# sclipman/gfa2network

Hardware: AMD Instinct MI355X
Metric: M edges/sec GFA->CSR (device-resident), + GB/s ingested (higher is better)
Workload: dtype u8/int64 (float64 weights); 1 GPU; C4: 50M S / 200M L, default (directed, MAX-SYM CSR), HBM-resident parse; n_segments=50000000, n_links=200000000, input_bytes_per_gpu=6299989066, n_nodes=50000000, nnz=289480899, mode=default, output=csr, parallelism=replica x1

## Files before the change

### gfa2network_amd/_native.py

```python
from __future__ import annotations

import ctypes
import os
import sys
from dataclasses import dataclass, field
from pathlib import Path

import numpy as np

LIB_PATH = Path(__file__).resolve().parent / "_lib" / "libg2n.so"

ABI_VERSION = 2
MAX_PHASES = 40

OK = 0
E_MALFORMED_L, E_MALFORMED_E, E_MALFORMED_C, E_MALFORMED_P, E_MALFORMED_O = 1, 2, 3, 4, 5
E_INDEX_LIST, E_INDEX_BYTES, E_UNICODE, E_INT_TOO_LARGE = 6, 7, 8, 9
E_CAST_OVERFLOW, E_CAST_INF, E_CAST_NAN = 10, 11, 12
E_ARG, E_IO, E_GZIP, E_DEVICE, E_NOMEM, E_UNSUPPORTED = 13, 14, 15, 16, 17, 18

DTYPE_CODES = {"bool": 0, "int8": 1, "int32": 2, "float32": 3, "float64": 4}
CODE_DTYPES = {v: np.dtype(k) for k, v in DTYPE_CODES.items()}
OUT_PARSE, OUT_CSR, OUT_COO, OUT_EDGE_LIST = 0, 1, 2, 3
FMT_COO, FMT_CSR, FMT_TEXT = 0, 1, 2

EXPORTED = [
    "g2n_version", "g2n_abi_version", "g2n_options_init", "g2n_device_count", "g2n_device_memory", "g2n_last_error",
    "g2n_status_name", "g2n_release_shared", "g2n_build_from_path", "g2n_build_from_buffer", "g2n_result_free",
    "g2n_coo_to_csr", "g2n_coo_to_csr_band", "g2n_context_create", "g2n_context_destroy", "g2n_context_stream", "g2n_context_trim",
    "g2n_build_device", "g2n_build_decimal_range", "g2n_count_device", "g2n_order_keys", "g2n_rank_keys", "g2n_upload_file_range", "g2n_partition_keys", "g2n_dedup_keys", "g2n_gather_keys", "g2n_remap_pairs", "g2n_route_triplets", "g2n_csr_from_coo_pair",
    "g2n_context_group_slots", "g2n_route_group_slots", "g2n_csr_from_group_slots",
    "g2n_keyset_create", "g2n_keyset_add", "g2n_keyset_view", "g2n_keyset_free",
    "g2n_gunzip", "g2n_gunzip_chunked", "g2n_free", "g2n_split_render", "g2n_split_get", "g2n_split_segments", "g2n_split_free", "g2n_join_names", "g2n_gather_names", "g2n_write_npz", "g2n_write_node_map", "g2n_first_bad_utf8",
    "g2n_csr_stats", "g2n_csr_stats_host", "g2n_stats_from_path",
    "g2n_csr_path_distances", "g2n_csr_path_distances_host", "g2n_load_paths", "g2n_paths_get", "g2n_paths_free",
    "g2n_distances_from_path", "g2n_csr_path_distances_weighted", "g2n_csr_path_distances_weighted_host",
    "g2n_seq_distance_from_path", "g2n_seq_hits_get", "g2n_seq_hits_names", "g2n_seq_hits_free",
]


TEST_NO_BUCKETS = 2
TEST_NO_LEAN = 4
TEST_DICT_HASH = 8
TEST_DICT_GENERAL = 16
TEST_NO_TILE_LOCAL = 32
TEST_HOST_INFLATE = 64
TEST_NO_GROUP = 128
TEST_NO_HASH_LEAN = 256
TEST_THROW_AFTER_IDS = 512
TEST_INDEX64 = 1024
TEST_DICT_DIRECT = 2048
TEST_NO_DIRECT = 4096
TEST_NO_EXT_LEAN = 8192
TEST_NO_DEC_TEXT = 16384
TEST_NO_DEC_PREFIX = 32768
TEST_FLAGS = int(os.environ.get("G2N_TEST_FLAGS", "0"), 0)
RANGE_DECIMAL = 1
RANGE_EVIDENCE = 2
RANGE_NO_VALUES = 4
RANGE_SLOTS = 8


class Options(ctypes.Structure):
    _fields_ = [
        ("abi_version", ctypes.c_uint32),
        ("directed", ctypes.c_int32),
        ("bidirected", ctypes.c_int32),
        ("keep_directed_bidir", ctypes.c_int32),
        ("asymmetric", ctypes.c_int32),
        ("strip_orientation", ctypes.c_int32),
        ("dtype", ctypes.c_int32),
        ("output", ctypes.c_int32),
        ("weight_tag", ctypes.c_char_p),
        ("want_node_names", ctypes.c_int32),
        ("device", ctypes.c_int32),
        ("unknown_warned", ctypes.c_int32),
        ("range_flags", ctypes.c_int32),
        ("range_s_base", ctypes.c_int64),
        ("range_n_segments", ctypes.c_int64),
        ("test_flags", ctypes.c_uint32),
        ("reserved_", ctypes.c_int32 * 3),
    ]


class Result(ctypes.Structure):
    _fields_ = [
        ("abi_version", ctypes.c_uint32),
        ("status", ctypes.c_int32),
        ("err_line", ctypes.c_int64),
        ("err_index", ctypes.c_int64),
        ("err_value", ctypes.c_double),
        ("err_detail", ctypes.c_void_p),
        ("err_detail_len", ctypes.c_int64),
        ("has_warning", ctypes.c_int32),
        ("warn_byte", ctypes.c_int32),
        ("warn_line", ctypes.c_int64),
        ("n_lines", ctypes.c_int64),
        ("n_records", ctypes.c_int64),
        ("n_records_before_error", ctypes.c_int64),
        ("n_edges", ctypes.c_int64),
        ("n_nodes", ctypes.c_int64),
        ("names_blob", ctypes.c_void_p),
        ("names_offsets", ctypes.c_void_p),
        ("format", ctypes.c_int32),
        ("dtype", ctypes.c_int32),
        ("index_width", ctypes.c_int32),
        ("sum_sorted", ctypes.c_int32),
        ("nnz", ctypes.c_int64),
# ... 291 lines not shown
    o.device = int(device)
    o.test_flags = int(TEST_FLAGS if test_flags is None else test_flags)
    return o


class _Owner:

    def __init__(self, ptr):
        self.ptr = ptr

    def __del__(self):
        if self.ptr is not None and _lib is not None:
            _lib.g2n_result_free(self.ptr)
            self.ptr = None


def _view(addr: int | None, count: int, dtype, owner: _Owner) -> np.ndarray:
    dtype = np.dtype(dtype)
    if not addr or count == 0:
        return np.zeros(0, dtype=dtype)
    buf = (ctypes.c_uint8 * (count * dtype.itemsize)).from_address(addr)
    buf._g2n_owner = owner
    return np.frombuffer(buf, dtype=dtype, count=count)


@dataclass
class RawResult:

    status: int = 0
    message: str = ""
    err_line: int = -1
    err_index: int = -1
    err_value: float = 0.0
    err_detail: bytes = b""
    has_warning: bool = False
    warn_byte: int = 0
    warn_line: int = -1
    n_lines: int = 0
    n_records: int = 0
    n_records_before_error: int = 0
    n_edges: int = 0
    n_nodes: int = 0
    names_blob: np.ndarray | None = None
    names_offsets: np.ndarray | None = None
    format: str = "coo"
    dtype: np.dtype = field(default_factory=lambda: np.dtype("float64"))
    rows: np.ndarray | None = None
    cols: np.ndarray | None = None
    indptr: np.ndarray | None = None
    indices: np.ndarray | None = None
    data: np.ndarray | None = None
    sum_sorted: bool = True
    sum_buckets: bool = False
    n_cast_overflow: int = 0
    input_bytes: int = 0
    phase_ms: dict = field(default_factory=dict)
    host_ms: dict = field(default_factory=dict)


def _from_result(ptr, rc: int) -> RawResult:
    if not ptr:
        raise RuntimeError(f"{status_name(rc)}: {last_error()}")
    r = ptr.contents
    owner = _Owner(ptr)
    out = RawResult(status=r.status, message=last_error() if r.status else "")
    out.err_line, out.err_index, out.err_value = r.err_line, r.err_index, r.err_value
    if r.err_detail and r.err_detail_len:
        out.err_detail = ctypes.string_at(r.err_detail, r.err_detail_len)
    out.has_warning, out.warn_byte, out.warn_line = bool(r.has_warning), r.warn_byte, r.warn_line
    out.n_lines, out.n_records = r.n_lines, r.n_records
    out.n_records_before_error, out.n_edges, out.n_nodes = r.n_records_before_error, r.n_edges, r.n_nodes
    out.dtype = CODE_DTYPES.get(r.dtype, np.dtype("float64"))
    out.sum_sorted = bool(r.sum_sorted)
    out.sum_buckets = r.sum_sorted < 0
    out.n_cast_overflow = int(r.n_cast_overflow)
    out.input_bytes = int(r.input_bytes)
    if r.format == FMT_TEXT and r.data:
        out.format = "text"
        out.data = _view(r.data, r.nnz, np.uint8, owner)
    elif r.status == OK:
        idx = np.int32 if r.index_width == 4 else np.int64
        if r.names_offsets:
            out.names_offsets = _view(r.names_offsets, r.n_nodes + 1, np.int64, owner)
            out.names_blob = _view(r.names_blob, int(out.names_offsets[-1]), np.uint8, owner)
        if r.format == FMT_COO:
            out.format = "coo"
            out.rows = _view(r.rows, r.nnz, idx, owner)
            out.cols = _view(r.cols, r.nnz, idx, owner)
        else:
            out.format = "csr"
            out.indptr = _view(r.indptr, r.n_nodes + 1, idx, owner)
            out.indices = _view(r.indices, r.nnz, idx, owner)
        out.data = _view(r.data, r.nnz, out.dtype, owner)
    for k in range(r.n_phases):
        name = r.phase_names[k].decode()
        if not name.startswith("_"):
            out.phase_ms[name] = out.phase_ms.get(name, 0.0) + r.phase_ms[k]
    out.host_ms = {"read": r.host_ms_read, "h2d": r.host_ms_h2d, "d2h": r.host_ms_d2h}
    return out


def build_from_path(path: str, opts: Options) -> RawResult:
    lib = load()
    res = ctypes.POINTER(Result)()
    rc = lib.g2n_build_from_path(os.fsencode(path), ctypes.byref(opts), ctypes.byref(res))
    return _from_result(res, rc)


def build_from_buffer(data: bytes | bytearray | memoryview | np.ndarray, opts: Options) -> RawResult:
    lib = load()
    arr = np.frombuffer(data, dtype=np.uint8) if not isinstance(data, np.ndarray) else data
    arr = np.ascontiguousarray(arr, dtype=np.uint8)
    res = ctypes.POINTER(Result)()
    rc = lib.g2n_build_from_buffer(arr.ctypes.data if arr.size else None, arr.size, ctypes.byref(opts),
                                   ctypes.byref(res))
    return _from_result(res, rc)


def _stats_dict(st: GraphStats) -> dict:
    return {"n_nodes": int(st.n_nodes), "n_entries": int(st.n_entries), "n_diag": int(st.n_diag),
            "n_components": int(st.n_components), "max_degree": int(st.max_degree),
            "ms_degree": float(st.ms_degree), "ms_components": float(st.ms_components)}


def stats_from_path(path: str, opts: Options) -> tuple[RawResult, dict, int]:
    lib = load()
    res = ctypes.POINTER(Result)()
# ... 494 lines not shown
```

### gfa2network_amd/csrc/g2n_kernels.h

```cpp
#pragma once
#include <hip/hip_runtime.h>
#include <stdint.h>

#include "stl_sort.h"

namespace g2n {

constexpr int kTPB = 256;
constexpr uint64_t kTile = 32768;
constexpr uint32_t kTileHalo = 2048;

enum : uint8_t { kSkip = 0, kUnknown = 1, kS = 2, kEdge = 3, kPO = 4 };

enum : uint32_t {
  kErrMalformedL = 1,
  kErrMalformedE = 2,
  kErrMalformedC = 3,
  kErrMalformedP = 4,
  kErrMalformedO = 5,
  kErrIndexList = 6,
  kErrIndexBytes = 7,
  kErrUnicode = 8,
  kErrIntTooLarge = 9,
  kErrCastOverflow = 10,
  kErrCastInf = 11,
  kErrCastNan = 12,
};

constexpr uint64_t kConstFlag = 1ull << 62;
constexpr unsigned long long kEmptySlot = ~0ull;

struct Ctl {
  unsigned long long err_key;
  unsigned long long warn_line;
  unsigned long long cast_key;
  unsigned long long wl_count;
  unsigned long long n_lines;
  unsigned long long n_records;
  unsigned long long n_edges;
  unsigned long long n_s;
  unsigned long long n_records_before;
  unsigned long long n_nodes;
  unsigned long long names_len;
  unsigned long long table_overflow;
  unsigned long long detail_off;
  unsigned long long detail_len;
  unsigned long long unsorted[2];
  unsigned long long flagged[2];
  unsigned long long n_unique[2];
  unsigned long long n_keep;
  unsigned long long n_f32_overflow;
  unsigned long long deferred;
  unsigned long long dict_general;
  unsigned long long s_late;
  unsigned long long row_gap;
  unsigned long long n_deferred;
  unsigned long long int_fail;
  unsigned long long bucket_overflow;
  unsigned long long bad_id;
  unsigned long long ev_dmin, ev_dmax;
  unsigned long long ev_vmax;
  unsigned long long w_inexact;
  unsigned long long warn_tile;
  unsigned long long warn_off;
  unsigned long long dir_vmax;
};

struct ParseOpts {
  int bidir, keep, strip, has_wt;
  uint32_t wt_len;
  const uint8_t* wt;
  uint32_t* tid;
  uint64_t n_seg;
  uint64_t s_base;
  int32_t* rows;
  int32_t* cols;
  uint32_t ktrip;
  uint32_t tile_pad;
  uint32_t grouped;
  double* ew;
  uint64_t wt_pack;
  uint32_t* tunk;
  uint64_t dpre;
  uint32_t dpre_len;
  uint32_t gshift;
  uint32_t* wenc;
  uint32_t wf32;
};
constexpr uint32_t kGroupShift = 5;

struct TileLean {
  long long dmin, dmax;
  unsigned long long vmax;
};

struct TouchOut {
  uint64_t* noff;
  uint32_t* nlen;
  uint64_t* ooff;
  uint32_t* olen;
  uint8_t* tkind;
};
struct DictEntry {
  unsigned long long hdr;
  unsigned long long meta;
  unsigned long long k0, k1;
};
struct TouchIn {
  const uint64_t* noff;
  const uint32_t* nlen;
  const uint64_t* ooff;
// ... 35 lines not shown
```

### gfa2network_amd/csrc/g2n_pipeline.hip

```cpp
#include <hip/hip_runtime.h>

#include <chrono>
#include <cstring>
#include <functional>
#include <map>
#include <memory>
#include <mutex>

#include "g2n_internal.h"
#include "g2n_kernels.hip"
#include "g2n_scan.hip"
#include "g2n_sort.hip"
#include "g2n_sym.hip"
#include "g2n_route.hip"
#include "g2n_inflate.hip"
#include "g2n_keyset.hip"
#include "g2n_stats.hip"
#include "g2n_dist.hip"
#include "g2n_wdist.hip"
#include "g2n_seq.hip"

#define G2N_HIP(call)                                                                                      \
  do {                                                                                                     \
    hipError_t e_ = (call);                                                                                \
    if (e_ != hipSuccess)                                                                                  \
      throw ::g2n::Failure(G2N_E_DEVICE, std::string(#call " failed: ") + hipGetErrorString(e_));          \
  } while (0)

namespace g2n {

enum Slot {
  S_IN, S_TILE_CNT, S_TILE_BASE, S_LS, S_KIND, S_NOFF, S_NLEN, S_OOFF, S_OLEN, S_EW, S_ETB, S_WL, S_TABLE,
  S_SLOT, S_FIRST, S_NID, S_FLEN, S_BLOB, S_OFFS, S_ROWS, S_COLS, S_DATA, S_KEYS0, S_KEYS1, S_VALS0, S_VALS1,
  S_KV, S_ODATA, S_INDPTR, S_INDICES, S_TEMP, S_WT, S_TKIND, S_TSTATE, S_RSTART0, S_RSTART1, S_ROUT0,
  S_ROUT1, S_UCNT0, S_UCNT1, S_UOFF, S_MCNT, S_MOFF, S_RSCR, S_RFLAG0, S_RFLAG1, S_RVAL0, S_RVAL1, S_TID,
  S_INV, S_TUNK, S_DEFER, S_FOFF64, S_BTC, S_BTV, S_BTOT, S_EBAD, S_ELEN, S_EPOS, S_ETEXT, S_EFIRST, S_EMETA, S_EL0, S_EL1,
  S_PCNT, S_POFF, S_PGRP, S_BSTART, S_SCANST, S_RBOUND, S_ROWSP, S_COLSP, S_TLEAN, S_ZIN, S_ZMEM, S_ZBAD, S_RSK, S_RSV, S_RSCNT, S_RSOFF,
  S_GCNT, S_TCN, S_INDPTR64, S_INDICES64, S_WENC, S_W1, S_W2, S_TVAL, S_PW0, S_PW1, S_BSTARTA, S_DIRECT, S_RTOT, S_SCANST2, S_EWP, S_TLIST, S_TNB, S_WENCP,
  S_STPARENT, S_STCOL, S_STDIAG, S_STLONG, S_STOUT, S_STIP, S_STIX,
  S_DSEEN, S_DNEXT, S_DQUEUE, S_DQMASK, S_DLONG, S_DSTATE, S_DCNT, S_DMPTR, S_DCUR, S_DMPATH, S_DSPATH, S_DDONE,
  S_DTAB, S_DPP, S_DPN,
  S_WDIST, S_WVAL,
  S_DFLAG, S_DKS, S_DSBLOB, S_DSOFFS, S_DIDS,
  S_QSTATE, S_QLINES, S_QNODE, S_QFPOS, S_QFLAG, S_QLAST, S_QCAND, S_QIDS, S_QBYTES, S_QNLEN, S_QNOFF, S_QNBLOB,
  S_NSLOTS
};

constexpr uint64_t kMinGroups = 1024;
constexpr uint32_t kPtileSmallDiv = 4;
constexpr uint32_t kF2Ranges = 4;
constexpr uint32_t kTestNoBuckets = G2N_TEST_NO_BUCKETS;
constexpr uint32_t kTestNoLean = G2N_TEST_NO_LEAN;
constexpr uint32_t kTestDictHash = G2N_TEST_DICT_HASH;
constexpr uint32_t kTestDictGeneral = G2N_TEST_DICT_GENERAL;
constexpr uint32_t kTestNoTileLocal = G2N_TEST_NO_TILE_LOCAL;
constexpr uint32_t kTestNoGroup = G2N_TEST_NO_GROUP;
constexpr uint32_t kTestNoHashLean = G2N_TEST_NO_HASH_LEAN;
constexpr uint32_t kTestThrowAfterIds = G2N_TEST_THROW_AFTER_IDS;
constexpr uint32_t kTestIndex64 = G2N_TEST_INDEX64;
constexpr uint32_t kTestDictDirect = G2N_TEST_DICT_DIRECT;
constexpr uint32_t kTestNoDirect = G2N_TEST_NO_DIRECT;
constexpr uint32_t kTestNoExtLean = G2N_TEST_NO_EXT_LEAN;
constexpr uint32_t kTestNoDecText = G2N_TEST_NO_DEC_TEXT;
constexpr uint32_t kTestNoDecPrefix = G2N_TEST_NO_DEC_PREFIX;


struct DevBuf {
  void* p = nullptr;
  size_t cap = 0;
  uint64_t call = 0;
};
struct ScanSlot {
  void* p = nullptr;
  size_t cap = 0;
  uint32_t epoch = 0;
  uint64_t ticket = 0;
};

struct GroupedCoo {
  bool active = false;
  bool failed = false;
  const int32_t* rows = nullptr;
  const int32_t* cols = nullptr;
  const uint32_t* gcount = nullptr;
  uint64_t gcap = 0, n_groups = 0;
  const uint32_t* wenc = nullptr;
};

}

struct g2n_context {
  int device = 0;
  int n_cu = 256;
  uint32_t test_flags = 0;
  uint64_t err_line_off = 0;
  g2n::GroupedCoo gcoo;
  g2n::GroupedCoo slots;
  const uint32_t* wenc = nullptr;
  bool no_group = false;
  g2n::ScanSlot scan_slot[g2n::S_NSLOTS];
  bool edge_text = false;
  bool names_dec = false;
  bool stats_names = false;
  uint64_t last_n_segs = 0;
  hipStream_t stream = nullptr;
  hipStream_t side = nullptr;
  hipEvent_t side_ev[2] = {nullptr, nullptr};
  hipStream_t place = nullptr;
  hipEvent_t ov_ev[17] = {};
  bool side_pending = false;
  bool range_has_s = false;
  int64_t range_d = -1;
  uint64_t range_vmax = 0;
  uint64_t range_nseg = 0;
  std::function<void()> side_work;
  std::vector<g2n::DevBuf> bufs;
  uint64_t call_id = 0;
// ... 362 lines not shown
    const uint64_t n_blk2 = (n_el + ptile - 1) / ptile + n_dig1;
    const uint64_t n2 = (uint64_t)n_dig2 * n_blk2;
    const uint64_t ns = words ? 2 : 1;
    auto* cnt2 = dget<uint32_t>(c, S_PCNT, ns * n2);
    auto* off2 = dget<uint32_t>(c, S_POFF, std::max<uint64_t>(ns * n2, ns * nm1));
    auto* el2 = dget<uint2>(c, S_EL1, n_el);
    PartSrc s2a{nullptr, nullptr, 0, 0, nullptr, nullptr, 0, 0, nullptr, grpA, grpA + n_dig1 + 1, n_dig1,
                nullptr, 0, (uint32_t)low + 1u, nullptr, wa1, ptile};
    s2a.obase = off2 + n2;
    uint16_t* wa2 = words ? dget<uint16_t>(c, S_PW1, n_trip) : nullptr;
    const bool wide = bits2 > (int)kMaxDigitBits;
    if (wide) {
      hipLaunchKernelGGL((k_part_hist<2, kWideDigitBits>), dim3((unsigned)n_blk2), dim3(kPartTPB), 0, c->stream, s2,
                         (uint32_t)low, n_dig2, cnt2, n_blk2);
      if (words)
        hipLaunchKernelGGL((k_part_hist<7, kWideDigitBits>), dim3((unsigned)n_blk2), dim3(kPartTPB), 0, c->stream,
                           s2a, 2u * (uint32_t)low, n_dig2, cnt2 + n2, n_blk2);
    } else {
      hipLaunchKernelGGL(k_part_hist<2>, dim3((unsigned)n_blk2), dim3(kPartTPB), 0, c->stream, s2, (uint32_t)low,
                         n_dig2, cnt2, n_blk2);
      if (words)
        hipLaunchKernelGGL(k_part_hist<7>, dim3((unsigned)n_blk2), dim3(kPartTPB), 0, c->stream, s2a,
                           2u * (uint32_t)low, n_dig2, cnt2 + n2, n_blk2);
    }
    scan_excl<uint32_t, uint32_t>(c, cnt2, off2, ns * n2);
    if (wide)
      hipLaunchKernelGGL((k_part_scatter<2, kWideDigitBits>), dim3((unsigned)n_blk2), dim3(kPartTPB), 0, c->stream, s2,
                         (uint32_t)low, n_dig2, (const uint32_t*)off2, n_blk2, el2);
    else
      hipLaunchKernelGGL(k_part_scatter<2>, dim3((unsigned)n_blk2), dim3(kPartTPB), 0, c->stream, s2, (uint32_t)low,
                         n_dig2, (const uint32_t*)off2, n_blk2, el2);
    hipLaunchKernelGGL(k_part_bucket_starts, dim3(grid_for(n_buckets + 1)), dim3(kTPB), 0, c->stream,
                       (const uint32_t*)off2, s2, n_dig2, n_buckets, bst);
    el = el2;
    if (words) {
      if (wide)
        hipLaunchKernelGGL((k_part_scatter<7, kWideDigitBits>), dim3((unsigned)n_blk2), dim3(kPartTPB), 0,
                           c->stream, s2a, 2u * (uint32_t)low, n_dig2, (const uint32_t*)(off2 + n2), n_blk2,
                           (uint2*)nullptr, (uint32_t*)wa2);
      else
        hipLaunchKernelGGL(k_part_scatter<7>, dim3((unsigned)n_blk2), dim3(kPartTPB), 0, c->stream, s2a,
                           2u * (uint32_t)low, n_dig2, (const uint32_t*)(off2 + n2), n_blk2, (uint2*)nullptr,
                           (uint32_t*)wa2);
      hipLaunchKernelGGL(k_part_bucket_starts, dim3(grid_for(n_buckets + 1)), dim3(kTPB), 0, c->stream,
                         (const uint32_t*)(off2 + n2), s2a, n_dig2, n_buckets, bstA);
      wa = wa2;
    }
  }
  phase(c, "sum");
  auto* indptr = dget<int32_t>(c, S_INDPTR, n_rows + 1);
  auto* indices = dget<int32_t>(c, S_INDICES, n_el);
  T* odata = dget<T>(c, S_ODATA, n_el);
  auto* btot = dget<uint32_t>(c, S_BTOT, n_bk);
  uint2* tmp = el == el1 ? dget<uint2>(c, S_EL1, n_el) : el1;
  auto* tcol = (uint32_t*)tmp;
  auto* tcn = dget<uint16_t>(c, S_TCN, 2 * n_el);
  G2N_HIP(hipMemsetAsync(&c->ctl->bucket_overflow, 0, sizeof(unsigned long long), c->stream));
#ifdef G2N_F1_STAMPS
  unsigned long long* f1st = dget<unsigned long long>(c, S_TEMP, n_bk * kF1Stamps);
  G2N_HIP(hipMemsetAsync(f1st, 0, n_bk * kF1Stamps * 8, c->stream));
  G2N_HIP(hipMemcpyToSymbolAsync(HIP_SYMBOL(g2n_f1_stamps), &f1st, sizeof(f1st), 0, hipMemcpyHostToDevice,
                                 c->stream));
#endif
  fork_side(c);
  const uint32_t n_ov = (n_el <= 0x7FFFFFFFull && !(c->test_flags & kTestIndex64) && n_bk >= 32768ull) ? kF2Ranges : 1u;
  auto rb = [&](uint32_t k) -> uint64_t { return n_bk * k / n_ov; };
  uint32_t* boff = nullptr;
  auto launch_f1 = [&](uint64_t b0, uint64_t nb) {
    auto* f1 = sum ? k_sym_finish<T, true> : k_sym_finish<T, false>;
    hipLaunchKernelGGL(f1, dim3((unsigned)nb), dim3(kFinTPB), 0, c->stream, el, (const uint32_t*)bst, (uint32_t)low,
                       n_rows, (T)1, btot, tcol, tcn, indptr, c->ctl, (uint32_t)row_base, wa, (const uint32_t*)bstA,
                       (uint32_t)b0);
  };
  auto launch_f2 = [&](hipStream_t st, auto* ind, int64_t* ip64, uint64_t b0, uint64_t nb, const uint32_t* rt,
                       uint32_t rk) {
    using I = std::remove_pointer_t<decltype(ind)>;
    hipLaunchKernelGGL((k_sym_place<T, I>), dim3((unsigned)nb), dim3(kFinTPB), 0, st, (const uint32_t*)bst,
                       (const uint32_t*)btot, (const uint32_t*)boff, (uint32_t)low, n_rows, (T)1, (const uint32_t*)tcol,
                       (const uint16_t*)tcn, indptr, ind, odata, ip64, (const uint32_t*)bstA, (uint32_t)b0, rt, rk);
  };
  if (n_ov > 1) {
    boff = dget<uint32_t>(c, S_MOFF, n_bk + 1);
    auto* rtot = dget<uint32_t>(c, S_RTOT, n_ov);
    (void)dget<unsigned long long>(c, S_SCANST2, scan_tiles(n_bk) + 1);
    for (uint32_t k = 0; k < n_ov; k++) {
      launch_f1(rb(k), rb(k + 1) - rb(k));
      G2N_HIP(hipEventRecord(c->ov_ev[k], c->stream));
    }
    for (uint32_t k = 0; k < n_ov; k++) {
      const uint64_t b0 = rb(k), b1 = rb(k + 1);
      G2N_HIP(hipStreamWaitEvent(c->place, c->ov_ev[k], 0));
      scan_excl<uint32_t, uint32_t>(c, (const uint32_t*)(btot + b0), boff + b0, b1 - b0, rtot + k, c->place, S_SCANST2);
      launch_f2(c->place, indices, nullptr, b0, b1 - b0, rtot, k);
    }
    G2N_HIP(hipEventRecord(c->ov_ev[16], c->place));
    G2N_HIP(hipStreamWaitEvent(c->stream, c->ov_ev[16], 0));
    int32_t nnz = 0;
    G2N_HIP(hipMemcpyAsync(&nnz, indptr + n_rows, sizeof(int32_t), hipMemcpyDeviceToHost, c->stream));
    sync_ctl(c);
#ifdef G2N_F1_STAMPS
    stamps_to_file(c, "G2N_F1_STAMPS_OUT", f1st, n_bk / n_ov * kF1Stamps);
#endif
    if (c->h_ctl->bucket_overflow) return false;
    R->format = G2N_FMT_CSR;
    R->indptr = indptr;
    R->nnz = (int64_t)nnz;
    R->indices = indices;
    R->data = odata;
    R->sum_sorted = -1;
    R->sum_t_sorted = -1;
    phase(c, sum ? "csr" : "maxsym");
    return true;
  }
  launch_f1(0, n_bk);
#ifdef G2N_F1_STAMPS
  stamps_to_file(c, "G2N_F1_STAMPS_OUT", f1st, n_bk * kF1Stamps);
#endif
  boff = dget<uint32_t>(c, S_MOFF, n_bk + 1);
  scan_excl<uint32_t, uint32_t>(c, btot, boff, n_bk, boff + n_bk);
  if (n_el > 0x7FFFFFFFull || (c->test_flags & kTestIndex64)) {
    sync_ctl(c);
    if (c->h_ctl->bucket_overflow) return false;
  }
  const bool wide = (c->test_flags & kTestIndex64) || (sum && !pair && n_trip > 0x7FFFFFFFull) ||
                    (!sum && n_el > 0x7FFFFFFFull && (uint64_t)read_dev(c, boff + n_bk) > 0x7FFFFFFFull);
  if (wide) {
// ... 2417 lines not shown
```

### gfa2network_amd/csrc/g2n_sym.hip

```cpp
#pragma once
#include <hip/hip_runtime.h>
#include <stdint.h>

#include <type_traits>

#include "g2n_kernels.h"
#include "g2n_scan.hip"
#include "g2n_symword.h"

namespace g2n {

constexpr uint32_t kPartTPB = 1024;
constexpr uint32_t kSubPer = 8;
constexpr uint32_t kSub = kSubPer * kPartTPB;
constexpr uint32_t kChunkSubs = 8 * 1024 / kPartTPB;
constexpr uint32_t kPartTile = kSub * kChunkSubs;
constexpr uint32_t kMaxDigitBits = 10;
constexpr uint32_t kWideDigitBits = 11;
constexpr uint32_t kFinTPB = 256;
static_assert(kFinTPB == 1u << kSymLowMax, "a finish bucket's row must fit the 8-bit fields of a 16-bit pair word");
constexpr uint32_t kSymCap = 16 * kFinTPB;
constexpr uint32_t kSymPer = kSymCap / kFinTPB;
constexpr uint32_t kSymReg = 8;

// ... 431 lines not shown

constexpr uint32_t kShortRow = 16;
constexpr uint32_t kMidRow = 64;
constexpr uint32_t kStagedSkip = 0xFFFFFFFFu;
constexpr uint32_t kMultiCopy = 0x80000000u;

__device__ inline uint32_t wave_sort64(uint32_t x) {
  const uint32_t lane = threadIdx.x & 63;
#pragma unroll
  for (uint32_t k = 2; k <= 64; k <<= 1)
#pragma unroll
    for (uint32_t j = k >> 1; j > 0; j >>= 1) {
      const uint32_t y = (uint32_t)__shfl_xor((int)x, (int)j, 64);
      const bool up = (lane & k) == 0;
      const bool lower = (lane & j) == 0;
      x = (lower == up) ? min(x, y) : max(x, y);
    }
  return x;
}

template <class Keep, class Emit>
__device__ inline uint32_t wave_merge(uint32_t x, uint32_t nr, Keep keep, Emit emit) {
  const uint32_t lane = threadIdx.x & 63;
  const uint32_t col = x >> 1, sd = x & 1u;
  const bool valid = lane < nr;
  const uint32_t pcol = (uint32_t)__shfl_up((int)col, 1, 64), ncol = (uint32_t)__shfl_down((int)col, 1, 64);
  const bool start = valid && (lane == 0 || pcol != col);
  const bool last = valid && (lane + 1 == nr || ncol != col);
  const unsigned long long smask = __ballot(start), s1 = __ballot(valid && sd);
  const unsigned long long upto = (2ull << lane) - 1ull;
  const uint32_t sl = 63u - (uint32_t)__clzll((smask & upto) | 1ull);
  const unsigned long long run = upto & ~((1ull << sl) - 1ull);
  const uint32_t ky = (uint32_t)__popcll(s1 & run), kx = lane - sl + 1 - ky;
  uint32_t kk = 0;
  const bool kept = last && keep(kx, ky, kk);
  const unsigned long long km = __ballot(kept);
  if (kept) emit((uint32_t)__popcll(km & ((1ull << lane) - 1ull)), col, kk);
  return (uint32_t)__popcll(km);
}

#ifdef G2N_F1_STAMPS
constexpr int kF1Stamps = 10;
__device__ unsigned long long* g2n_f1_stamps;
#define F1_STAMP(k)                                                                          \
  do {                                                                                       \
    if (threadIdx.x == 0) g2n_f1_stamps[blockIdx.x * kF1Stamps + (k)] = wall_clock64();      \
  } while (0)
#else
#define F1_STAMP(k) \
  do {              \
  } while (0)
#endif

template <class T, bool kSum>
__global__ void __launch_bounds__(kFinTPB) __attribute__((amdgpu_waves_per_eu(8, 8))) k_sym_finish(const uint2* __restrict__ el, const uint32_t* __restrict__ bstart,
                                                     uint32_t low, uint64_t n_rows, T one, uint32_t* __restrict__ btot,
                                                     uint32_t* __restrict__ tcol, uint16_t* __restrict__ tcn,
                                                     int32_t* __restrict__ indptr, Ctl* ctl, uint32_t row_base, const uint16_t* __restrict__ wa,
                                                     const uint32_t* __restrict__ bstA, uint32_t b0) {
  __shared__ __attribute__((aligned(16))) uint32_t seg[kSymCap];
  __shared__ uint32_t cnt[kFinTPB];
  __shared__ uint32_t cur[kFinTPB];
  __shared__ uint32_t red[kFinTPB / 64];
  __shared__ uint16_t mlist[kFinTPB];
  __shared__ uint32_t mval[kFinTPB];
  __shared__ uint32_t mcount;
  F1_STAMP(0);
  cnt[threadIdx.x] = 0;
  if (threadIdx.x == 0) mcount = 0;
  const uint64_t b = b0 + blockIdx.x;
  const uint32_t eB = bstart[b], nB = bstart[b + 1] - eB;
  const uint32_t eA = bstA ? bstA[b] : 0u, nA = bstA ? bstA[b + 1] - eA : 0u;
  const uint32_t e0 = eB + eA, n = nB + nA;
  auto overflow = [&]() {
    if (threadIdx.x == 0) {
      ctl->bucket_overflow = 1;
      btot[b] = 0;
    }
  };
  if (n > kSymCap) {
    overflow();
    return;
  }
  __syncthreads();
  const uint32_t rmask = (1u << low) - 1u;
  uint32_t my, rs, nx;
  {
    auto word = [&](uint32_t w) {
      uint32_t ra, rb;
      sym_word_rows(w, (uint32_t)b, low, &ra, &rb);
      return make_uint2(ra, ((rb + row_base) << 2) | kElPair);
    };
    const uint32_t nr = bstA ? nA : nB;
    uint2 xs[kSymReg];
    uint2 xb = make_uint2(0, 0);
    if (bstA) {
      uint32_t ws[kSymReg];
#pragma unroll
      for (uint32_t k = 0; k < kSymReg; k++) {
        const uint32_t i = threadIdx.x + k * kFinTPB;
        ws[k] = i < nr ? wa[eA + i] : 0u;
      }
      if (threadIdx.x < nB) xb = el[eB + threadIdx.x];
#pragma unroll
      for (uint32_t k = 0; k < kSymReg; k++) xs[k] = word(ws[k]);
    } else {
#pragma unroll
      for (uint32_t k = 0; k < kSymReg; k++) {
        const uint32_t i = threadIdx.x + k * kFinTPB;
        if (i < nr) xs[k] = el[eB + i];
      }
    }
    auto count = [&](uint2 x) {
      atomicAdd(&cnt[x.x & rmask], 1u);
      if ((x.y & 3u) == kElPair) atomicAdd(&cnt[((x.y >> 2) - row_base) & rmask], 1u);
    };
    auto place = [&](uint2 x) {
      const uint32_t kind = x.y & 3u, col = x.y >> 2;
      seg[atomicAdd(&cur[x.x & rmask], 1u)] = (col << 1) | (kind & 1u);
      if (kind == kElPair)
        seg[atomicAdd(&cur[(col - row_base) & rmask], 1u)] = ((x.x + row_base) << 1) | (kSum ? 0u : 1u);
    };
#pragma unroll
// ... 61 lines not shown
    }
  };
  uint32_t kmask = 0;
  uint64_t kq[kShortRow / 8] = {};
  auto short_merge = [&]() -> uint32_t {
    uint32_t kx = 0, ky = 0;
#pragma unroll
    for (uint32_t q = 0; q < kShortRow; q++) {
      const bool valid = q < my;
      const uint32_t sd = k[q] & 1u;
      kx += (valid && !sd) ? 1u : 0u;
      ky += (valid && sd) ? 1u : 0u;
      const bool last = valid && (q + 1 == kShortRow || (k[q + 1] >> 1) != (k[q] >> 1));
      uint32_t kk;
      const bool kept = keep(kx, ky, kk);
      kmask |= (last && kept) ? 1u << q : 0u;
      kq[q / 8] |= (uint64_t)(kk & 0xFFu) << (8 * (q % 8));
      kx = last ? 0u : kx;
      ky = last ? 0u : ky;
    }
    return (uint32_t)__builtin_popcount(kmask);
  };
  auto long_merge = [&](auto emit) -> uint32_t {
    uint32_t i = 0, m = 0;
    while (i < my) {
      const uint32_t c = sg[i] >> 1;
      uint32_t kx = 0, ky = 0;
      while (i < my && (sg[i] >> 1) == c) {
        if (sg[i] & 1) ky++;
        else kx++;
        i++;
      }
      uint32_t kk;
      if (keep(kx, ky, kk)) emit(m++, c, kk);
    }
    return m;
  };
  auto none = [](uint32_t, uint32_t, uint32_t) {};
  if (n_mid) {
    for (uint32_t i = wv; i < n_mid; i += kFinTPB / 64) {
      const uint32_t r = mlist[i], s0 = cnt[r], nr = cur[r] - s0;
      uint32_t x = lane < nr ? seg[s0 + lane] : 0xFFFFFFFFu;
      x = wave_sort64(x);
      if (lane < nr) seg[s0 + lane] = x;
      const uint32_t mm = wave_merge(x, nr, keep, none);
      if (lane == 0) mval[r] = mm;
    }
    __syncthreads();
  }
  F1_STAMP(3);
  const uint32_t m = !live ? 0u : (shortrow ? short_merge() : midrow ? mval[threadIdx.x] : long_merge(none));
  uint32_t off;
  const uint32_t tot = block_excl_scan_n<kFinTPB>(m, &off, red);
  if (threadIdx.x == 0) btot[b] = tot;
  F1_STAMP(4);
  uint32_t* ocol = tcol + 2 * (uint64_t)e0;
  uint16_t* ocn = tcn + 2 * (uint64_t)e0;
  auto stage = [&](uint32_t j, uint32_t c, uint32_t kk) -> uint32_t {
    if (kk > 1u) ocn[j] = (uint16_t)kk;
    return kk > 1u ? (c | kMultiCopy) : c;
  };
  auto out = [&](uint32_t j, uint32_t c, uint32_t kk) { ocol[j] = stage(j, c, kk); };
  if (live) {
    indptr[row] = (int32_t)off;
    if (row == n_rows - 1) indptr[n_rows] = (int32_t)(off + m);
    if (longrow)
      long_merge([&](uint32_t j, uint32_t c, uint32_t kk) { out(off + j, c, kk); });
    if (midrow) mval[threadIdx.x] = off;
  }
  __syncthreads();
  if (n_mid) {
    for (uint32_t i = wv; i < n_mid; i += kFinTPB / 64) {
      const uint32_t r = mlist[i], s0 = cnt[r], nr = cur[r] - s0, o = mval[r];
      const uint32_t x = lane < nr ? seg[s0 + lane] : 0xFFFFFFFFu;
      wave_merge(x, nr, keep, [&](uint32_t j, uint32_t c, uint32_t kk) { out(o + j, c, kk); });
    }
    __syncthreads();
  }
  if (live) {
    if (shortrow) {
      uint32_t j = off;
#pragma unroll
      for (uint32_t q = 0; q < kShortRow; q++)
        if (kmask >> q & 1u) {
          seg[j] = stage(j, k[q] >> 1, (uint32_t)(kq[q / 8] >> (8 * (q % 8))) & 0xFFu);
          j++;
        }
    } else {
      for (uint32_t j = 0; j < m; j++) seg[off + j] = kStagedSkip;
    }
  }
  __syncthreads();
  F1_STAMP(5);
  for (uint32_t i = threadIdx.x; i < tot; i += kFinTPB) {
    const uint32_t c = seg[i];
    if (c == kStagedSkip) continue;
    ocol[i] = c;
  }
#ifdef G2N_F1_STAMPS
  F1_STAMP(6);
  if (threadIdx.x == 0) {
    uint32_t hw, xcc;
    asm volatile("s_getreg_b32 %0, hwreg(HW_REG_HW_ID)" : "=s"(hw));
    asm volatile("s_getreg_b32 %0, hwreg(HW_REG_XCC_ID)" : "=s"(xcc));
    g2n_f1_stamps[blockIdx.x * kF1Stamps + 9] = ((unsigned long long)xcc << 32) | hw;
  }
#endif
}

template <class T, class I>
__global__ void __launch_bounds__(kFinTPB) k_sym_place(const uint32_t* __restrict__ bstart, const uint32_t* __restrict__ btot,
                                                    const uint32_t* __restrict__ boff, uint32_t low, uint64_t n_rows,
                                                    T one, const uint32_t* __restrict__ tcol,
                                                    const uint16_t* __restrict__ tcn, int32_t* __restrict__ indptr,
                                                    I* __restrict__ indices, T* __restrict__ data,
                                                    int64_t* __restrict__ indptr64, const uint32_t* __restrict__ bstA,
                                                    uint32_t b0, const uint32_t* __restrict__ rtot, uint32_t rk) {
  const uint32_t b = b0 + blockIdx.x;
  uint32_t rbase = 0;
  for (uint32_t j = 0; rtot && j < rk; j++) rbase += rtot[j];
  const uint32_t e0 = bstart[b] + (bstA ? bstA[b] : 0u), tot = btot[b], base = boff[b] + rbase;
  const uint32_t* src = tcol + 2 * (uint64_t)e0;
  const uint16_t* scn = tcn + 2 * (uint64_t)e0;
  constexpr uint32_t kU = 8;
  for (uint32_t i0 = threadIdx.x; i0 < tot; i0 += kU * kFinTPB) {
    uint32_t c[kU];
#pragma unroll
    for (uint32_t u = 0; u < kU; u++) c[u] = i0 + u * kFinTPB < tot ? src[i0 + u * kFinTPB] : 0u;
#pragma unroll
    for (uint32_t u = 0; u < kU; u++) {
      const uint32_t i = i0 + u * kFinTPB;
      if (i < tot) {
        indices[(uint64_t)base + i] = (I)(c[u] & ~kMultiCopy);
        data[(uint64_t)base + i] = sum_copies<T>(one, (c[u] & kMultiCopy) ? (uint32_t)scn[i] : 1u);
      }
    }
  }
  const uint64_t row = ((uint64_t)b << low) + threadIdx.x;
  if (threadIdx.x < (1u << low) && row < n_rows) {
    if constexpr (sizeof(I) == 8) {
      indptr64[row] = (int64_t)base + (int64_t)(uint32_t)indptr[row];
      if (row == n_rows - 1) indptr64[n_rows] = (int64_t)base + (int64_t)(uint32_t)indptr[n_rows];
    } else {
      indptr[row] += (int32_t)base;
      if (row == n_rows - 1) indptr[n_rows] += (int32_t)base;
    }
  }
}


// ... 327 lines not shown
```

### include/g2n.h

```cpp
#ifndef G2N_H
#define G2N_H

#include <stddef.h>
#include <stdint.h>

#define G2N_VERSION_STRING "0.3.0"

#ifdef __cplusplus
extern "C" {
#endif

#define G2N_ABI_VERSION 2u

enum {
  G2N_OK = 0,
  G2N_E_MALFORMED_L = 1,
  G2N_E_MALFORMED_E = 2,
  G2N_E_MALFORMED_C = 3,
  G2N_E_MALFORMED_P = 4,
  G2N_E_MALFORMED_O = 5,
  G2N_E_INDEX_LIST = 6,
  G2N_E_INDEX_BYTES = 7,
  G2N_E_UNICODE = 8,
  G2N_E_INT_TOO_LARGE = 9,
// ... 5 lines not shown
  G2N_E_GZIP = 15,
  G2N_E_DEVICE = 16,
  G2N_E_NOMEM = 17,
  G2N_E_UNSUPPORTED = 18
};

enum { G2N_BOOL = 0, G2N_INT8 = 1, G2N_INT32 = 2, G2N_FLOAT32 = 3, G2N_FLOAT64 = 4 };

enum { G2N_OUT_PARSE = 0, G2N_OUT_CSR = 1, G2N_OUT_COO = 2, G2N_OUT_EDGE_LIST = 3 };
enum { G2N_FMT_COO = 0, G2N_FMT_CSR = 1, G2N_FMT_TEXT = 2 };

typedef struct g2n_options {
  uint32_t abi_version;
  int32_t directed;
  int32_t bidirected;
  int32_t keep_directed_bidir;
  int32_t asymmetric;
  int32_t strip_orientation;
  int32_t dtype;
  int32_t output;
  const char *weight_tag;
  int32_t want_node_names;
  int32_t device;
  int32_t unknown_warned;
  int32_t range_flags;
  int64_t range_s_base;
  int64_t range_n_segments;
  uint32_t test_flags;
  int32_t reserved_[3];
} g2n_options;

enum {
  G2N_RANGE_DECIMAL = 1,
  G2N_RANGE_EVIDENCE = 2,
  G2N_RANGE_NO_VALUES = 4,
  G2N_RANGE_SLOTS = 8
};

enum {
  G2N_TEST_NO_BUCKETS = 2,
  G2N_TEST_NO_LEAN = 4,
  G2N_TEST_DICT_HASH = 8,
  G2N_TEST_DICT_GENERAL = 16,
  G2N_TEST_NO_TILE_LOCAL = 32,
  G2N_TEST_HOST_INFLATE = 64,
  G2N_TEST_NO_GROUP = 128,
  G2N_TEST_NO_HASH_LEAN = 256,
  G2N_TEST_THROW_AFTER_IDS = 512,
  G2N_TEST_INDEX64 = 1024,
  G2N_TEST_DICT_DIRECT = 2048,
  G2N_TEST_NO_DIRECT = 4096,
  G2N_TEST_NO_EXT_LEAN = 8192,
  G2N_TEST_NO_DEC_TEXT = 16384,
  G2N_TEST_NO_DEC_PREFIX = 32768
};

#define G2N_MAX_PHASES 40

typedef struct g2n_result {
  uint32_t abi_version;
  int32_t status;
  int64_t err_line;
  int64_t err_index;
  double err_value;
  const uint8_t *err_detail;
  int64_t err_detail_len;
  int32_t has_warning;
  int32_t warn_byte;
  int64_t warn_line;
  int64_t n_lines;
  int64_t n_records;
  int64_t n_records_before_error;
  int64_t n_edges;
  int64_t n_nodes;
  const uint8_t *names_blob;
  const int64_t *names_offsets;
  int32_t format;
  int32_t dtype;
  int32_t index_width;
  int32_t sum_sorted;
  int64_t nnz;
  const void *rows;
  const void *cols;
  const void *indptr;
  const void *indices;
  const void *data;
  uint64_t names_bytes;
  int64_t n_cast_overflow;
  uint64_t input_bytes;
  int32_t n_phases;
  int32_t sum_t_sorted;
  double phase_ms[G2N_MAX_PHASES];
  const char *phase_names[G2N_MAX_PHASES];
  double host_ms_read;
  double host_ms_h2d;
  double host_ms_d2h;
  void *priv_;
} g2n_result;

const char *g2n_version(void);
uint32_t g2n_abi_version(void);
void g2n_options_init(g2n_options *opts);
int g2n_device_count(void);
int g2n_device_memory(int32_t device, uint64_t *free_bytes, uint64_t *total_bytes);
int g2n_release_shared(int32_t device, uint64_t *freed);
const char *g2n_last_error(void);
const char *g2n_status_name(int status);
// ... 173 lines not shown
```

Before: 27400 M edge records/s.

## Add count-then-place direct MAX-SYM finish writing CSR without staging

For the non-sum MAX-SYM path, a new k_sym_count kernel first counts the distinct cells in each bucket using a per-wave shared-memory bitmap. An exclusive scan turns those counts into output offsets, and a k_sym_finish variant then writes indices and data straight into the final CSR arrays. This drops the intermediate tcol/tcn staging buffers and the later placement pass. In exchange it adds an extra counting pass and a host sync, and it falls back to the old path when the count is declined or does not match the finish's own total.

```diff
diff --git a/gfa2network_amd/_native.py b/gfa2network_amd/_native.py
--- a/gfa2network_amd/_native.py
+++ b/gfa2network_amd/_native.py
@@ -54,6 +54,7 @@
 TEST_NO_EXT_LEAN = 8192
 TEST_NO_DEC_TEXT = 16384
 TEST_NO_DEC_PREFIX = 32768
+TEST_NO_DIRECT_FINISH = 65536
 TEST_FLAGS = int(os.environ.get("G2N_TEST_FLAGS", "0"), 0)
 RANGE_DECIMAL = 1
 RANGE_EVIDENCE = 2
@@ -451,6 +452,7 @@
     data: np.ndarray | None = None
     sum_sorted: bool = True
     sum_buckets: bool = False
+    sym_direct: bool = False
     n_cast_overflow: int = 0
     input_bytes: int = 0
     phase_ms: dict = field(default_factory=dict)
@@ -472,6 +474,7 @@
     out.dtype = CODE_DTYPES.get(r.dtype, np.dtype("float64"))
     out.sum_sorted = bool(r.sum_sorted)
     out.sum_buckets = r.sum_sorted < 0
+    out.sym_direct = r.sum_t_sorted == -2
     out.n_cast_overflow = int(r.n_cast_overflow)
     out.input_bytes = int(r.input_bytes)
     if r.format == FMT_TEXT and r.data:
diff --git a/gfa2network_amd/csrc/g2n_kernels.h b/gfa2network_amd/csrc/g2n_kernels.h
--- a/gfa2network_amd/csrc/g2n_kernels.h
+++ b/gfa2network_amd/csrc/g2n_kernels.h
@@ -57,6 +57,8 @@
   unsigned long long n_deferred;
   unsigned long long int_fail;
   unsigned long long bucket_overflow;
+  unsigned long long sym_decline;
+  unsigned long long sym_mismatch;
   unsigned long long bad_id;
   unsigned long long ev_dmin, ev_dmax;
   unsigned long long ev_vmax;
diff --git a/gfa2network_amd/csrc/g2n_pipeline.hip b/gfa2network_amd/csrc/g2n_pipeline.hip
--- a/gfa2network_amd/csrc/g2n_pipeline.hip
+++ b/gfa2network_amd/csrc/g2n_pipeline.hip
@@ -63,6 +63,7 @@
 constexpr uint32_t kTestNoExtLean = G2N_TEST_NO_EXT_LEAN;
 constexpr uint32_t kTestNoDecText = G2N_TEST_NO_DEC_TEXT;
 constexpr uint32_t kTestNoDecPrefix = G2N_TEST_NO_DEC_PREFIX;
+constexpr uint32_t kTestNoDirectFinish = G2N_TEST_NO_DIRECT_FINISH;
 
 
 struct DevBuf {
@@ -531,10 +532,18 @@
   auto* indices = dget<int32_t>(c, S_INDICES, n_el);
   T* odata = dget<T>(c, S_ODATA, n_el);
   auto* btot = dget<uint32_t>(c, S_BTOT, n_bk);
-  uint2* tmp = el == el1 ? dget<uint2>(c, S_EL1, n_el) : el1;
-  auto* tcol = (uint32_t*)tmp;
-  auto* tcn = dget<uint16_t>(c, S_TCN, 2 * n_el);
-  G2N_HIP(hipMemsetAsync(&c->ctl->bucket_overflow, 0, sizeof(unsigned long long), c->stream));
+  const bool direct = !sum && !pair && n_el <= 0x7FFFFFFFull && !std::is_same<T, int8_t>::value &&
+                      !(c->test_flags & (kTestIndex64 | kTestNoDirectFinish));
+  uint32_t* tcol = nullptr;
+  uint16_t* tcn = nullptr;
+  auto staging = [&]() {
+    uint2* tmp = el == el1 ? dget<uint2>(c, S_EL1, n_el) : el1;
+    tcol = (uint32_t*)tmp;
+    tcn = dget<uint16_t>(c, S_TCN, 2 * n_el);
+  };
+  static_assert(offsetof(Ctl, sym_mismatch) == offsetof(Ctl, bucket_overflow) + 2 * sizeof(unsigned long long),
+                "the finish's three flags are cleared together");
+  G2N_HIP(hipMemsetAsync(&c->ctl->bucket_overflow, 0, 3 * sizeof(unsigned long long), c->stream));
 #ifdef G2N_F1_STAMPS
   unsigned long long* f1st = dget<unsigned long long>(c, S_TEMP, n_bk * kF1Stamps);
   G2N_HIP(hipMemsetAsync(f1st, 0, n_bk * kF1Stamps * 8, c->stream));
@@ -549,8 +558,44 @@
     auto* f1 = sum ? k_sym_finish<T, true> : k_sym_finish<T, false>;
     hipLaunchKernelGGL(f1, dim3((unsigned)nb), dim3(kFinTPB), 0, c->stream, el, (const uint32_t*)bst, (uint32_t)low,
                        n_rows, (T)1, btot, tcol, tcn, indptr, c->ctl, (uint32_t)row_base, wa, (const uint32_t*)bstA,
-                       (uint32_t)b0);
+                       (uint32_t)b0, (const uint32_t*)nullptr, (int32_t*)nullptr, (T*)nullptr);
   };
+  if (direct) {
+    boff = dget<uint32_t>(c, S_MOFF, n_bk + 1);
+    static const int cnt_per_cu = [] {
+      int n = 0;
+      if (hipOccupancyMaxActiveBlocksPerMultiprocessor(&n, k_sym_count, 64 * kCntWaves, 0) != hipSuccess || n < 1) n = 1;
+      return n;
+    }();
+    const uint64_t cnt_blocks =
+        std::min<uint64_t>((n_bk + kCntWaves - 1) / kCntWaves, (uint64_t)cnt_per_cu * (uint64_t)c->n_cu);
+    hipLaunchKernelGGL(k_sym_count, dim3((unsigned)cnt_blocks), dim3(64 * kCntWaves), 0, c->stream, el,
+                       (const uint32_t*)bst, wa, (const uint32_t*)bstA, (uint32_t)low, (uint32_t)n_bk, n_buckets, btot,
+                       c->ctl);
+    scan_excl<uint32_t, uint32_t>(c, btot, boff, n_bk);
+    hipLaunchKernelGGL((k_sym_finish<T, false, true>), dim3((unsigned)n_bk), dim3(kFinTPB), 0, c->stream, el,
+                       (const uint32_t*)bst, (uint32_t)low, n_rows, (T)1, btot, (uint32_t*)nullptr, (uint16_t*)nullptr,
+                       indptr, c->ctl, 0u, wa, (const uint32_t*)bstA, 0u, (const uint32_t*)boff, indices, odata);
+    int32_t nnz = 0;
+    G2N_HIP(hipMemcpyAsync(&nnz, indptr + n_rows, sizeof(int32_t), hipMemcpyDeviceToHost, c->stream));
+    sync_ctl(c);
+#ifdef G2N_F1_STAMPS
+    stamps_to_file(c, "G2N_F1_STAMPS_OUT", f1st, n_bk * kF1Stamps);
+#endif
+    if (c->h_ctl->bucket_overflow || c->h_ctl->sym_mismatch) return false;
+    if (!c->h_ctl->sym_decline) {
+      R->format = G2N_FMT_CSR;
+      R->indptr = indptr;
+      R->nnz = (int64_t)nnz;
+      R->indices = indices;
+      R->data = odata;
+      R->sum_sorted = -1;
+      R->sum_t_sorted = -2;
+      phase(c, "maxsym");
+      return true;
+    }
+  }
+  staging();
   auto launch_f2 = [&](hipStream_t st, auto* ind, int64_t* ip64, uint64_t b0, uint64_t nb, const uint32_t* rt,
                        uint32_t rk) {
     using I = std::remove_pointer_t<decltype(ind)>;
diff --git a/gfa2network_amd/csrc/g2n_sym.hip b/gfa2network_amd/csrc/g2n_sym.hip
--- a/gfa2network_amd/csrc/g2n_sym.hip
+++ b/gfa2network_amd/csrc/g2n_sym.hip
@@ -507,12 +507,126 @@
   } while (0)
 #endif
 
-template <class T, bool kSum>
+constexpr uint32_t kCntWaves = 4;
+constexpr uint32_t kCntMapWords = (1u << (2 * kSymLowMax)) / 32u;
+constexpr uint32_t kCntQ = 4;
+constexpr uint32_t kCntBPer = kFinTPB / 64;
+
+__global__ void __launch_bounds__(64 * kCntWaves) k_sym_count(const uint2* __restrict__ el, const uint32_t* __restrict__ bstart,
+                                                             const uint16_t* __restrict__ wa, const uint32_t* __restrict__ bstA,
+                                                             uint32_t low, uint32_t n_bk, uint64_t n_buckets,
+                                                             uint32_t* __restrict__ btot, Ctl* ctl) {
+  __shared__ uint4 map4[kCntWaves][kCntMapWords / 4];
+  __shared__ unsigned long long bkey[kCntWaves][kFinTPB];
+  if (bstart[n_buckets] > bstA[n_buckets]) {
+    if (blockIdx.x == 0 && threadIdx.x == 0) ctl->sym_decline = 1;
+    return;
+  }
+  const uint32_t lane = threadIdx.x & 63, wv = threadIdx.x >> 6;
+  uint32_t* map = (uint32_t*)map4[wv];
+  unsigned long long* bk = bkey[wv];
+  const uint32_t rmask = (1u << low) - 1u;
+  const uint32_t map_q = (((1u << (2 * low)) + 31u) / 32u + 3u) / 4u;
+  const uint32_t stride = gridDim.x * kCntWaves;
+  struct Ahead {
+    uint32_t eA, nA, eB, nB;
+    uint4 ws[kCntQ];
+    uint2 xb;
+  };
+  const uint4* wa4 = (const uint4*)wa;
+  auto q0_of = [](const Ahead& h) { return h.eA >> 3; };
+  auto nq_of = [](const Ahead& h) { return h.nA ? ((h.eA + h.nA + 7u) >> 3) - (h.eA >> 3) : 0u; };
+  auto starts = [&](uint32_t b, Ahead& h) {
+    h.eA = h.nA = h.eB = h.nB = 0;
+    if (b < n_bk) {
+      h.eA = bstA[b];
+      h.nA = bstA[b + 1] - h.eA;
+      h.eB = bstart[b];
+      h.nB = bstart[b + 1] - h.eB;
+    }
+  };
+  auto fetch = [&](Ahead& h) {
+    const uint32_t q0 = q0_of(h), nq = nq_of(h);
+#pragma unroll
+    for (uint32_t k = 0; k < kCntQ; k++) {
+      const uint32_t i = lane + 64u * k;
+      h.ws[k] = i < nq ? wa4[q0 + i] : make_uint4(0, 0, 0, 0);
+    }
+    h.xb = lane < h.nB ? el[h.eB + lane] : make_uint2(0, 0);
+  };
+  uint32_t b = blockIdx.x * kCntWaves + wv;
+  Ahead cur, nxt;
+  starts(b, cur);
+  fetch(cur);
+  starts(b + stride, nxt);
+  for (; b < n_bk; b += stride) {
+    Ahead n2;
+    fetch(nxt);
+    starts(b + 2 * stride, n2);
+    const bool over = cur.nA + cur.nB > kSymCap;
+    const bool wide = cur.nB > kFinTPB;
+    if (wide && !over && lane == 0) ctl->sym_decline = 1;
+    uint32_t cells = 0;
+    if (!over && !wide) {
+      for (uint32_t i = lane; i < map_q; i += 64) map4[wv][i] = make_uint4(0, 0, 0, 0);
+      __builtin_amdgcn_fence(__ATOMIC_RELEASE, "wavefront");
+      __builtin_amdgcn_wave_barrier();
+      auto word = [&](uint32_t w) {
+        const uint32_t ra = (w >> low) & rmask, rb = w & rmask;
+        const uint32_t lo = ra < rb ? ra : rb, hi = ra < rb ? rb : ra;
+        const uint32_t key = (lo << low) | hi, bit = 1u << (key & 31u);
+        if (!(atomicOr(&map[key >> 5], bit) & bit)) cells += lo != hi ? 2u : 1u;
+      };
+      const uint32_t q0 = q0_of(cur), nq = nq_of(cur), wend = cur.eA + cur.nA;
+      auto piece = [&](uint4 v, uint32_t q) {
+        const uint32_t u[4] = {v.x, v.y, v.z, v.w};
+#pragma unroll
+        for (uint32_t j = 0; j < 8; j++) {
+          const uint32_t i = 8u * q + j;
+          if (i >= cur.eA && i < wend) word((u[j >> 1] >> (16u * (j & 1u))) & 0xFFFFu);
+        }
+      };
+#pragma unroll
+      for (uint32_t k = 0; k < kCntQ; k++)
+        if (lane + 64u * k < nq) piece(cur.ws[k], q0 + lane + 64u * k);
+      for (uint32_t i = lane + 64u * kCntQ; i < nq; i += 64) piece(wa4[q0 + i], q0 + i);
+      uint2 xs[kCntBPer];
+#pragma unroll
+      for (uint32_t q = 0; q < kCntBPer; q++) {
+        const uint32_t i = lane + 64u * q;
+        xs[q] = q == 0 ? cur.xb : (i < cur.nB ? el[cur.eB + i] : make_uint2(0, 0));
+        if (i < cur.nB) bk[i] = ((unsigned long long)xs[q].x << 32) | (xs[q].y >> 2);
+      }
+      __builtin_amdgcn_fence(__ATOMIC_RELEASE, "wavefront");
+      __builtin_amdgcn_wave_barrier();
+#pragma unroll
+      for (uint32_t q = 0; q < kCntBPer; q++) {
+        const uint32_t i = lane + 64u * q;
+        if (i < cur.nB) {
+          const unsigned long long me = ((unsigned long long)xs[q].x << 32) | (xs[q].y >> 2);
+          bool dup = false;
+          for (uint32_t j = 0; j < i; j++) dup |= bk[j] == me;
+          cells += dup ? 0u : 1u;
+        }
+      }
+      __builtin_amdgcn_wave_barrier();
+    }
+    for (int o = 32; o > 0; o >>= 1) cells += (uint32_t)__shfl_xor((int)cells, o, 64);
+    if (lane == 0) btot[b] = cells;
+    cur = nxt;
+    nxt = n2;
+  }
+}
+
+template <class T, bool kSum, bool kDirect = false>
 __global__ void __launch_bounds__(kFinTPB) __attribute__((amdgpu_waves_per_eu(8, 8))) k_sym_finish(const uint2* __restrict__ el, const uint32_t* __restrict__ bstart,
                                                      uint32_t low, uint64_t n_rows, T one, uint32_t* __restrict__ btot,
                                                      uint32_t* __restrict__ tcol, uint16_t* __restrict__ tcn,
                                                      int32_t* __restrict__ indptr, Ctl* ctl, uint32_t row_base, const uint16_t* __restrict__ wa,
-                                                     const uint32_t* __restrict__ bstA, uint32_t b0) {
+                                                     const uint32_t* __restrict__ bstA, uint32_t b0,
+                                                     const uint32_t* __restrict__ boff, int32_t* __restrict__ indices,
+                                                     T* __restrict__ data) {
+  static_assert(!(kSum && kDirect), "the finish in place is MAX-SYM's");
   __shared__ __attribute__((aligned(16))) uint32_t seg[kSymCap];
   __shared__ uint32_t cnt[kFinTPB];
   __shared__ uint32_t cur[kFinTPB];
@@ -524,6 +638,12 @@
   cnt[threadIdx.x] = 0;
   if (threadIdx.x == 0) mcount = 0;
   const uint64_t b = b0 + blockIdx.x;
+  uint32_t base = 0, given = 0;
+  if constexpr (kDirect) {
+    if (ctl->sym_decline) return;
+    base = boff[b];
+    given = btot[b];
+  }
   const uint32_t eB = bstart[b], nB = bstart[b + 1] - eB;
   const uint32_t eA = bstA ? bstA[b] : 0u, nA = bstA ? bstA[b + 1] - eA : 0u;
   const uint32_t e0 = eB + eA, n = nB + nA;
@@ -691,18 +811,34 @@
   const uint32_t m = !live ? 0u : (shortrow ? short_merge() : midrow ? mval[threadIdx.x] : long_merge(none));
   uint32_t off;
   const uint32_t tot = block_excl_scan_n<kFinTPB>(m, &off, red);
-  if (threadIdx.x == 0) btot[b] = tot;
+  if constexpr (kDirect) {
+    if (threadIdx.x == 0 && tot != given) ctl->sym_mismatch = 1;
+  } else {
+    if (threadIdx.x == 0) btot[b] = tot;
+  }
   F1_STAMP(4);
-  uint32_t* ocol = tcol + 2 * (uint64_t)e0;
-  uint16_t* ocn = tcn + 2 * (uint64_t)e0;
+  uint32_t* ocol = kDirect ? nullptr : tcol + 2 * (uint64_t)e0;
+  uint16_t* ocn = kDirect ? nullptr : tcn + 2 * (uint64_t)e0;
+  int32_t* oind = kDirect ? indices + base : nullptr;
+  T* odat = kDirect ? data + base : nullptr;
   auto stage = [&](uint32_t j, uint32_t c, uint32_t kk) -> uint32_t {
-    if (kk > 1u) ocn[j] = (uint16_t)kk;
+    if (kk > 1u) {
+      if constexpr (kDirect) odat[j] = sum_copies<T>(one, kk);
+      else ocn[j] = (uint16_t)kk;
+    }
     return kk > 1u ? (c | kMultiCopy) : c;
   };
-  auto out = [&](uint32_t j, uint32_t c, uint32_t kk) { ocol[j] = stage(j, c, kk); };
+  auto out = [&](uint32_t j, uint32_t c, uint32_t kk) {
+    if constexpr (kDirect) {
+      oind[j] = (int32_t)c;
+      odat[j] = sum_copies<T>(one, kk);
+    } else {
+      ocol[j] = stage(j, c, kk);
+    }
+  };
   if (live) {
-    indptr[row] = (int32_t)off;
-    if (row == n_rows - 1) indptr[n_rows] = (int32_t)(off + m);
+    indptr[row] = (int32_t)(base + off);
+    if (row == n_rows - 1) indptr[n_rows] = (int32_t)(base + off + m);
     if (longrow)
       long_merge([&](uint32_t j, uint32_t c, uint32_t kk) { out(off + j, c, kk); });
     if (midrow) mval[threadIdx.x] = off;
@@ -734,7 +870,12 @@
   for (uint32_t i = threadIdx.x; i < tot; i += kFinTPB) {
     const uint32_t c = seg[i];
     if (c == kStagedSkip) continue;
-    ocol[i] = c;
+    if constexpr (kDirect) {
+      oind[i] = (int32_t)(c & ~kMultiCopy);
+      if (!(c & kMultiCopy)) odat[i] = one;
+    } else {
+      ocol[i] = c;
+    }
   }
 #ifdef G2N_F1_STAMPS
   F1_STAMP(6);
diff --git a/include/g2n.h b/include/g2n.h
--- a/include/g2n.h
+++ b/include/g2n.h
@@ -81,7 +81,8 @@
   G2N_TEST_NO_DIRECT = 4096,
   G2N_TEST_NO_EXT_LEAN = 8192,
   G2N_TEST_NO_DEC_TEXT = 16384,
-  G2N_TEST_NO_DEC_PREFIX = 32768
+  G2N_TEST_NO_DEC_PREFIX = 32768,
+  G2N_TEST_NO_DIRECT_FINISH = 65536
 };
 
 #define G2N_MAX_PHASES 40
```

Result: faster. 29380 M edge records/s (median of 6 runs) (+7.2%).
